# decadenza/SimpleStereo

Measured on AMD Instinct MI355X. Metric: disparity MPixels/s (H*W*nDisp per second), higher is better.
Workload: dtype f32

## Files before the change

simplestereo_amd/csrc/asw_pipe_kernel.hip.h:

```cpp
#pragma once
#include "asw_kernels.hip.h"
#ifndef SSAMD_KERNEL_TU
#include "lab_kernels.hip.h"
#endif

namespace ssamd {

#ifndef SSAMD_KERNEL_TU
static constexpr int TADV_COLS = 64;
template <bool BYTES>
__device__ __forceinline__ void asw_tad_tile(const void *__restrict__ srcL, const void *__restrict__ srcR, unsigned char *__restrict__ evol,
                                             int W, int pad, int minD, int Dc, int Se, int erow0, int erows, int evolW, int rd, long long npix_total,
                                             int bx, int by, int bz, char *smem)
{
    uint32_t *const sL = reinterpret_cast<uint32_t *>(smem);
    uint32_t *const sR = sL + TADV_COLS;
    const int r = erow0 + by, z = bz, uc0 = bx * TADV_COLS;
    const int P = Se >> 2, dlo = minD + z * Dc, dhi = dlo + Dc - 1;
    const int u0 = uc0 - pad, xr0 = u0 - dhi;
    auto pixel = [&](const void *src, int col) -> uint32_t {
        const size_t q = (size_t)r * W + col;
        if constexpr (BYTES) {
            typedef uint32_t __attribute__((aligned(1))) u32_unaligned;
            const uint8_t *const b = reinterpret_cast<const uint8_t *>(src) + 3 * q;
            return (long long)q + 1 < npix_total ? (*reinterpret_cast<const u32_unaligned *>(b) & 0xffffffu)
                                                 : ((uint32_t)b[0] | ((uint32_t)b[1] << 8) | ((uint32_t)b[2] << 16));
        } else {
            return reinterpret_cast<const PixRec *>(src)[q].bgrx;
        }
    };
    for (int k = threadIdx.x; k < 2 * TADV_COLS + Dc; k += blockDim.x) {
        const bool isL = k < TADV_COLS;
        const int col = isL ? u0 + k : xr0 + (k - TADV_COLS);
        const uint32_t v = (unsigned)col < (unsigned)W ? pixel(isL ? srcL : srcR, col) : 0x80000000u;
        (isL ? sL : sR)[isL ? k : k - TADV_COLS] = v;
    }
    __syncthreads();
    const int ncols = min(TADV_COLS, evolW - uc0);
    uint32_t *const out = reinterpret_cast<uint32_t *>(evol + (((size_t)z * erows + by) * (size_t)evolW + uc0) * Se);
    auto dword = [&](int c, int slot, uint32_t lp) {
        uint32_t v = 0;
        const int d0 = rd == 6 ? 6 * (slot >> 1) + 4 * (slot & 1) : 4 * slot, nv = rd == 6 && (slot & 1) ? 2 : 4;
        if (!(lp >> 31) && d0 < Dc) {
            const uint32_t *const rp = sR + c + (Dc - 1) - d0;
#pragma unroll
            for (int q = 0; q < 4; ++q) {
                const uint32_t rv = q < nv && d0 + q < Dc ? rp[-q] : 0x80000000u;
                if (!(rv >> 31)) v |= min(__builtin_amdgcn_sad_u8(lp, rv, 0u), 40u) << (8 * q);
            }
        }
        return v;
    };
    if ((P & 3) == 0) {
        const int P4 = P >> 2;
        uint4 *const out4 = reinterpret_cast<uint4 *>(out);
        for (int k = threadIdx.x; k < ncols * P4; k += blockDim.x) {
            const int c = k / P4, s4 = 4 * (k - c * P4);
            const uint32_t lp = sL[c];
            out4[k] = make_uint4(dword(c, s4, lp), dword(c, s4 + 1, lp), dword(c, s4 + 2, lp), dword(c, s4 + 3, lp));
        }
        return;
    }
    for (int k = threadIdx.x; k < ncols * P; k += blockDim.x) {
        const int c = k / P, slot = k - c * P;
        out[k] = dword(c, slot, sL[c]);
    }
}

__global__ __launch_bounds__(256) void asw_tad_volume_kernel(const PixRec *__restrict__ recL, const PixRec *__restrict__ recR,
                                                             unsigned char *__restrict__ evol, int W, int pad, int minD, int Dc,
                                                             int Se, int erow0, int erows, int evolW, int rd = 4)
{
    extern __shared__ __attribute__((aligned(16))) char smem[];
    asw_tad_tile<false>(recL, recR, evol, W, pad, minD, Dc, Se, erow0, erows, evolW, rd, 0, blockIdx.x, blockIdx.y, blockIdx.z, smem);
}

struct AswPrepassArgs {
    const uint8_t *bgrL, *bgrR;
    PixRec *recL, *recR;
    unsigned char *evol;
    long long npix_total;
    int W, pad, minD, Dc, Se, erow0, erows, evolW, rd;
    int lab_blocks, ex, ey;
};
__global__ __launch_bounds__(256) void asw_prepass_kernel(const AswPrepassArgs P)
{
    extern __shared__ __attribute__((aligned(16))) char smem[];
    if ((int)blockIdx.x < P.lab_blocks) {
        SSAMD_LAB_TABLES_IN_LDS(T)
        const long long np = (long long)P.erows * P.W, first = (long long)P.erow0 * P.W;
        const uint8_t *const bl = P.bgrL + 3 * first, *const br = P.bgrR + 3 * first;
        PixRec *const rl = P.recL + first, *const rr = P.recR + first;
        typedef uint32_t __attribute__((aligned(1))) u32_unaligned;
        for (long long q = (long long)blockIdx.x * blockDim.x + threadIdx.x; q < 2 * np; q += (long long)P.lab_blocks * blockDim.x) {
            const bool right = q >= np;
            const long long p = right ? q - np : q;
            const uint8_t *const bgr = right ? br : bl;
            uint32_t B, G, R;
            if (p + 1 < np) {
                const uint32_t v = *reinterpret_cast<const u32_unaligned *>(bgr + 3 * p);
                B = v & 0xff; G = (v >> 8) & 0xff; R = (v >> 16) & 0xff;
            } else {
                B = bgr[3 * p]; G = bgr[3 * p + 1]; R = bgr[3 * p + 2];
            }
            PixRec o;
            bgr_to_lab(B, G, R, o.L, o.a, o.b, T);
            o.bgrx = B | (G << 8) | (R << 16);
            (right ? rr : rl)[p] = o;
        }
        return;
    }
    const int b = (int)blockIdx.x - P.lab_blocks, bx = b % P.ex, by = (b / P.ex) % P.ey, bz = b / (P.ex * P.ey);
    asw_tad_tile<true>(P.bgrL, P.bgrR, P.evol, P.W, P.pad, P.minD, P.Dc, P.Se, P.erow0, P.erows, P.evolW, P.rd, P.npix_total, bx, by, bz, smem);
}

#endif

template <bool WITH_COSTS, int SLC = 0, int SRC = 0, int SEC = 0, bool CG = false>
__global__ __launch_bounds__(ASW_MAX_THREADS, 3) void asw_aggregate_pipe_kernel(const AswArgs A)
{
    constexpr bool STATIC = SLC > 0;
    static_assert(!CG || STATIC, "compile-time geometry belongs to a static tile");
    constexpr int RX = ASW_RX;
    constexpr int NWR = asw_nwr(RX);
    extern __shared__ __attribute__((aligned(16))) char smem[];
    constexpr AswGeom SG = asw_pipe_geom_constexpr(AswPipeTile<SLC, SRC, SEC>::id);
    static_assert(!STATIC || (SG.SL == SLC && SG.SR == SRC && SG.Se == SEC), "the strides name the tile");
    const AswGeom &g = CG ? SG : A.g;
    float *const wL = reinterpret_cast<float *>(smem + g.off_wL);
    float *const wR = reinterpret_cast<float *>(smem + g.off_wR);
    unsigned char *const eT0 = reinterpret_cast<unsigned char *>(smem + g.off_e);
    float4 *const labL = reinterpret_cast<float4 *>(smem + g.off_labL);
    float4 *const labR = reinterpret_cast<float4 *>(smem + g.off_labR);
    uint32_t *const bgrL = reinterpret_cast<uint32_t *>(smem + g.off_bgrL);
    uint32_t *const bgrR = reinterpret_cast<uint32_t *>(smem + g.off_bgrR);
    u64 *const bestL = reinterpret_cast<u64 *>(smem + g.off_bestL);
    u64 *const bestR = reinterpret_cast<u64 *>(smem + g.off_bestR);
    float4 *const cenLab = reinterpret_cast<float4 *>(smem + g.off_cen);
    float *const proxS = reinterpret_cast<float *>(smem + g.off_prox);

    const int tid = threadIdx.x, nthr = blockDim.x;
    const int W = A.W, win = CG ? AswPipeTile<SLC, SRC, SEC>::id.win : A.win, p = CG ? AswPipeTile<SLC, SRC, SEC>::id.win / 2 : A.pad;
    const int Tx = g.Tx, Dc = g.Dc, nL = g.nL, nR = g.nR, nRc = g.nRc, SR = g.SR, Se = g.Se;
    const int JC = g.JC, NC = g.NC;
    int bx = blockIdx.x;
    if ((gridDim.x & 7) == 0) bx = (bx & 7) * (gridDim.x >> 3) + (bx >> 3);
    const int x0 = bx * Tx;
    const int y = asw_out_row(A, blockIdx.y);
    const int dlo = A.minD + blockIdx.z * Dc;
    const int dhi = dlo + Dc - 1;
    if (min(x0 + Tx - 1, W - 1) - dlo < 0) {
        if (A.disp)
            for (int k = threadIdx.x; k < Tx && x0 + k < W; k += blockDim.x)
                A.disp[(size_t)(y - A.row0) * W + x0 + k] = (int16_t)(x0 + k);
        return;
    }
    const int segL_lo = x0 - p, xrc_lo = x0 - dhi, segR_lo = xrc_lo - p;
    const int phase = g.dephase ? __builtin_amdgcn_readfirstlane((int)(threadIdx.x >> 8)) : 1;

    float accN[RX][ASW_RD], accS[RX][ASW_RD];
#pragma unroll
    for (int a = 0; a < RX; ++a)
#pragma unroll
        for (int b = 0; b < ASW_RD; ++b) { accN[a][b] = 0.f; accS[a][b] = 0.f; }

    for (int k = tid; k < Tx; k += nthr) bestL[k] = KEY_NONE;
    for (int k = tid; k <= nRc; k += nthr) bestR[k] = KEY_NONE;
    for (int c = tid; c < Tx + nRc; c += nthr) {
        const bool isL = c < Tx;
        const int ccol = isL ? x0 + c : xrc_lo + (c - Tx);
        float4 v = make_float4(0.f, 0.f, 0.f, 0.f);
        if ((unsigned)ccol < (unsigned)W) {
            const PixRec q = (isL ? A.recL : A.recR)[(size_t)y * W + ccol];
            v = make_float4(q.L, q.a, q.b, 1.f);
        }
        cenLab[c] = v;
    }

    const int i_lo = max(0, p - y), i_hi = min(win, A.H + p - y);

    auto stage_row = [&](int i) {
        int tids = threadIdx.x;
        asm volatile("" : "+v"(tids));
        const int buf = i & 1, r = y - p + i;
        for (int k = tids; k < win; k += nthr) proxS[buf * win + k] = A.prox[i * win + k];
        const PixRec *const rowL = A.recL + (size_t)r * W;
        const PixRec *const rowR = A.recR + (size_t)r * W;
        for (int k = tids; k < nL + nR; k += nthr) {
            const bool isL = k < nL;
            const int idx = isL ? k : k - nL;
            const int col = (isL ? segL_lo : segR_lo) + idx;
            PixRec v;
            v.L = __builtin_inff();
            v.a = v.b = 0.f;
            v.bgrx = 0u;
            if ((unsigned)col < (unsigned)W) v = (isL ? rowL : rowR)[col];
            (isL ? labL + buf * nL : labR + buf * nR)[idx] = make_float4(v.L, v.a, v.b, 0.f);
            if (!A.evol) (isL ? bgrL + buf * nL : bgrR + buf * nR)[idx] = v.bgrx;
        }
    };
    auto build_e = [&](int i, int t_lo, int t_hi) {
        int tidb = threadIdx.x;
        asm volatile("" : "+v"(tidb));
        unsigned char *const eT = eT0 + (i & 1) * g.e_bytes;
        const uint32_t *const bgrLc = bgrL + (i & 1) * nL, *const bgrRc = bgrR + (i & 1) * nR;
        const int e_q = nthr / nL, e_r = nthr - e_q * nL;
        int t = t_lo + tidb;
        int sp = t / nL, ul = t - sp * nL;
        while (t < t_hi) {
            const uint32_t lp = bgrLc[ul];
            const uint32_t *const rp = bgrRc + (ul + (Dc - 1) - 8 * sp);
            uint32_t lo = 0, hi = 0;
#pragma unroll
            for (int k = 0; k < 4; ++k) {
                lo |= min(__builtin_amdgcn_sad_u8(lp, rp[-k], 0u), 40u) << (8 * k);
                hi |= min(__builtin_amdgcn_sad_u8(lp, rp[-4 - k], 0u), 40u) << (8 * k);
            }
            uint32_t *const dst = reinterpret_cast<uint32_t *>(eT + ul * Se) + 2 * sp;
            dst[0] = lo;
            if (2 * sp + 1 < g.DG) dst[1] = hi;
            t += nthr; ul += e_r; sp += e_q;
            if (ul >= nL) { ul -= nL; ++sp; }
        }
    };
    auto load_e = [&](int i) {
        int tidd = threadIdx.x;
        asm volatile("" : "+v"(tidd));
        const int r = y - p + i;
        const unsigned char *const src = A.evol + (((size_t)blockIdx.z * A.erows + (r - A.erow0)) * (size_t)A.evolW + x0) * Se;
        unsigned char *const dst = eT0 + (i & 1) * g.e_bytes;
        const int bytes = nL * Se, lane16 = (tidd & 63) * 16;
        for (int k = __builtin_amdgcn_readfirstlane(tidd >> 6) * 1024; k < bytes; k += (nthr >> 6) * 1024)
            if (k + lane16 < bytes)
                __builtin_amdgcn_global_load_lds((const void *)(src + k + lane16),
                                                 (__attribute__((address_space(3))) void *)(dst + k), 16, 0, 0);
    };
    auto build_weights = [&](int i, int jb, int je, int rb) {
        int tidw = threadIdx.x;
        asm volatile("" : "+v"(tidw));
        const float4 *const labLc = labL + (i & 1) * nL, *const labRc = labR + (i & 1) * nR;
        const float *const prow = proxS + (i & 1) * win;
        const int ncen = Tx + nRc;
        const int full = ncen / nthr * nthr, rest = ncen - full;
        int slen = je - jb, nseg = 1;
        if (rest > 0 && full > 0) {
            slen = max(ASW_WB, (je - jb + nthr / rest - 1) / (nthr / rest));
            slen = (slen + ASW_WB - 1) / ASW_WB * ASW_WB;
            nseg = (je - jb + slen - 1) / slen;
        }
        const int ntasks = full + rest * nseg;
        for (int t = tidw; t < ntasks; t += nthr) {
            int c = t, jb_t = jb, je_t = je;
            if (t >= full && nseg > 1) {
                const int q = t - full, sgm = q / rest;
                c = full + q - sgm * rest;
                jb_t = jb + sgm * slen;
                je_t = min(je, jb_t + slen);
            }
            const bool isL = c < Tx;
            const int cc = isL ? c : c - Tx;
            const float4 cen = cenLab[c];
            const float4 *const seg = (isL ? labLc : labRc) + cc;
            const int stride = isL ? g.SL : SR;
            float *const wout = (isL ? wL : wR) + cc + (rb - jb) * stride;
            int j = jb_t;
            const float4 *sp = seg + j;
            const float *pp = prow + j;
            float *wp = wout + j * stride;
            const int stride4 = ASW_WB * stride;
            for (; j + ASW_WB <= je_t; j += ASW_WB, sp += ASW_WB, pp += ASW_WB, wp += stride4) {
                float4 tp[ASW_WB];
                float pr[ASW_WB], wv[ASW_WB];
#pragma unroll
                for (int u = 0; u < ASW_WB; ++u) { tp[u] = sp[u]; pr[u] = pp[u]; }
#pragma unroll
                for (int u = 0; u < ASW_WB; ++u) {
                    asm volatile("" ::"v"(tp[u].w));
                    const float dL = tp[u].x - cen.x, da = tp[u].y - cen.y, db = tp[u].z - cen.z;
                    wv[u] = fmaf(db, db, fmaf(da, da, dL * dL));
                }
#pragma unroll
                for (int u = 0; u < ASW_WB; ++u) wv[u] = __builtin_amdgcn_sqrtf(wv[u]);
#pragma unroll
                for (int u = 0; u < ASW_WB; ++u) wv[u] = asw_weight_finish(wv[u], A.kC, pr[u]);
#pragma unroll
                for (int u = 0; u < ASW_WB; ++u) wp[u * stride] = wv[u];
            }
            if (j < je_t) {
                float4 tp[ASW_WB];
                float pr[ASW_WB], wv[ASW_WB];
#pragma unroll
                for (int u = 0; u < ASW_WB; ++u) {
                    const int jj = min(j + u, je_t - 1);
                    tp[u] = seg[jj];
                    pr[u] = prow[jj];
                }
#pragma unroll
                for (int u = 0; u < ASW_WB; ++u) {
                    asm volatile("" ::"v"(tp[u].w));
                    const float dL = tp[u].x - cen.x, da = tp[u].y - cen.y, db = tp[u].z - cen.z;
                    wv[u] = fmaf(db, db, fmaf(da, da, dL * dL));
                }
#pragma unroll
                for (int u = 0; u < ASW_WB; ++u) wv[u] = __builtin_amdgcn_sqrtf(wv[u]);
#pragma unroll
                for (int u = 0; u < ASW_WB; ++u) wv[u] = asw_weight_finish(wv[u], A.kC, pr[u]);
#pragma unroll
                for (int u = 0; u < ASW_WB; ++u) {
                    const int jj = min(j + u, je_t - 1);
                    wout[jj * stride] = wv[u];
                }
            }
        }
    };
    auto chunk_end = [&](int c) { return c == NC - 1 ? win : (c + 1) * JC; };
    const int nE = nL * ((g.DG + 1) >> 1);
    auto build_next = [&](int i, int c, int cb) {
        const bool more_rows = i + 1 < i_hi;
        if (c == 0 && more_rows) stage_row(i + 1);
        if (c == 0 && more_rows && A.evol) load_e(i + 1);
        if (c + 1 < NC) build_weights(i, (c + 1) * JC, chunk_end(c + 1), (cb ^ 1) * g.JCmax);
        else if (more_rows) build_weights(i + 1, 0, chunk_end(0), (cb ^ 1) * g.JCmax);
        if (c >= 1 && more_rows && !A.evol) build_e(i + 1, (int)((long long)nE * (c - 1) / (NC - 1)), (int)((long long)nE * c / (NC - 1)));
    };

    stage_row(i_lo);
    if (A.evol) load_e(i_lo);
    __syncthreads();
    if (!A.evol) build_e(i_lo, 0, nE);
    build_weights(i_lo, 0, chunk_end(0), 0);

    const int DGe = max(1, min(g.DG, (min(min(x0 + Tx, W) - 1, x0 + Tx - 1) - dlo) / ASW_RD + 1));
    const int nact = g.XG * DGe;
    int pk_xd;
    bool run;
    {
        const int tidm = threadIdx.x;
        int xg, dg;
        const int F = DGe >> 4, Lo = DGe & 15, nfull = g.XG * F;
        const int grp16 = tidm >> 4, r16 = tidm & 15;
        if (grp16 < nfull) {
            xg = grp16 / F;
            int gi = grp16 - xg * F;
            if (xg & 1) gi = F - 1 - gi;
            dg = 16 * gi + r16;
        } else {
            const int q = tidm - 16 * nfull;
            xg = Lo ? q / Lo : g.XG;
            dg = 16 * F + (Lo ? q - xg * Lo : 0);
        }
        pk_xd = xg | (dg << 16);
        const bool tile_live = tidm < nact && x0 + RX * xg < W && dlo + ASW_RD * dg <= A.maxD &&
                               x0 + RX * xg + RX - 1 - (dlo + ASW_RD * dg) >= 0;
        run = __builtin_amdgcn_ballot_w64(tile_live) != 0 && tidm < nact;
    }

    int cb = 0;
#pragma nounroll
    for (int i = i_lo; i < i_hi; ++i) {
        const unsigned char *const eT = eT0 + (i & 1) * g.e_bytes;
        AswRow ew[RX];

#pragma nounroll
        for (int c = 0; c < NC; ++c) {
            __syncthreads();
            const int jc = c * JC, jend = chunk_end(c);
            const int rb = cb * g.JCmax;
            if (phase == 0) build_next(i, c, cb);
            if (run) {
                const int xg = pk_xd & 0xffff, dg = pk_xd >> 16;
                const unsigned char *erow = eT + (RX * xg + (jc == 0 ? 0 : RX - 1 + jc)) * Se + 4 * dg;
                if (jc == 0) {
#pragma unroll
                    for (int n = 0; n < RX - 1; ++n) {
                        asw_row_unpack(ew[n], *reinterpret_cast<const uint32_t *>(erow));
                        erow += Se;
                    }
                }
                const float *wlp = wL + rb * g.SL + 8 * xg;
                const float *wrp = wR + rb * SR + (RX * xg - ASW_RD * dg + Dc - ASW_RD);
                for (int j0 = jc; j0 < jend; j0 += RX) {
#define SSAMD_PSTEP(JJ)                                                                             \
    if (j0 + (JJ) < jend) {                                                                         \
        const uint32_t epk = *reinterpret_cast<const uint32_t *>(erow + (STATIC ? (JJ) * SEC : 0)); \
        if constexpr (!STATIC) erow += Se;                                                          \
        float wl[RX], wr[NWR];                                                                      \
        {                                                                                           \
            const float *const wl_ = wlp + (STATIC ? (JJ) * SLC : 0);                              \
            const float *const wr_ = wrp + (STATIC ? (JJ) * SRC : 0);                              \
            const float4 v0 = *reinterpret_cast<const float4 *>(wl_);                              \
            wl[0] = v0.x; wl[1] = v0.y; wl[2] = v0.z; wl[3] = v0.w;                                 \
            const float4 v1 = *reinterpret_cast<const float4 *>(wl_ + 4);                          \
            wl[4] = v1.x; wl[5] = v1.y; wl[6] = v1.z; wl[7] = v1.w;                                 \
            const float4 r0 = *reinterpret_cast<const float4 *>(wr_);                              \
            const float4 r1 = *reinterpret_cast<const float4 *>(wr_ + 4);                          \
            const float4 r2 = *reinterpret_cast<const float4 *>(wr_ + 8);                          \
            asm volatile("" ::"v"(r2.w));       \
            wr[0] = r0.x; wr[1] = r0.y; wr[2] = r0.z; wr[3] = r0.w;                                 \
            wr[4] = r1.x; wr[5] = r1.y; wr[6] = r1.z; wr[7] = r1.w;                                 \
            wr[8] = r2.x; wr[9] = r2.y; wr[10] = r2.z; wr[11] = r2.w;                               \
        }                                                                                           \
        if constexpr (!STATIC) { wlp += g.SL; wrp += SR; }                                         \
               \
        _Pragma("unroll") for (int xi = 0; xi < RX; ++xi) {                                         \
            if (xi == RX - 1) asw_row_unpack(ew[((JJ) + RX - 1) % RX], epk);                        \
            const AswRow &row_ = ew[((JJ) + xi) % RX];                                              \
            _Pragma("unroll") for (int di = 0; di < ASW_RD; ++di) {                                 \
                const float w_ = wl[xi] * wr[xi - di + ASW_RD - 1];                                 \
                accN[xi][di] = fmaf(w_, row_.e[di], accN[xi][di]);                                  \
                accS[xi][di] = fmaf(w_, row_.c[di], accS[xi][di]);                                  \
            }                                                                                       \
        }                                                                                           \
    }
                    SSAMD_PSTEP(0) SSAMD_PSTEP(1) SSAMD_PSTEP(2) SSAMD_PSTEP(3)
                    SSAMD_PSTEP(4) SSAMD_PSTEP(5) SSAMD_PSTEP(6) SSAMD_PSTEP(7)
#undef SSAMD_PSTEP
                    if constexpr (STATIC) { erow += RX * SEC; wlp += RX * SLC; wrp += RX * SRC; }
                }
            }
            if (phase != 0) build_next(i, c, cb);
            cb ^= 1;
        }
    }

    int tidf = threadIdx.x;
    asm volatile("" : "+v"(tidf));
#define ASW_EPI_RD ASW_RD
#define ASW_EPI_LIVE (tidf < nact)
#define ASW_EPI_XG(live) (pk_xd & 0xffff)
#define ASW_EPI_DG(live) (pk_xd >> 16)
#define ASW_EPI_TX Tx
#define ASW_EPI_NRC nRc
#define ASW_EPI_TID tid
#define ASW_EPI_NTHR nthr
#define ASW_EPI_SYNC() __syncthreads()
#define ASW_EPI_ROW (size_t)(y - A.row0) * W
#include "asw_epilogue.inc"
}

}
```

Baseline: 10650.

## Assign weight-build work per wavefront and read proximity weights from constant memory

Weight construction now distributes whole 64-lane wavefront columns of centres (left and right separately) instead of flat thread tasks. This keeps left/right branching uniform per wave, uses compile-time strides for static tiles and replaces the clamped remainder with exact 1-3 element batches. The proximity row is no longer staged into shared memory. It is read directly through the constant address space (scalar loads), which removes an LDS copy per row. The risks are heavier integer loop bookkeeping for task splitting and possibly worse load balance when the centre count does not fill the waves.

```diff
diff --git a/simplestereo_amd/csrc/asw_pipe_kernel.hip.h b/simplestereo_amd/csrc/asw_pipe_kernel.hip.h
--- a/simplestereo_amd/csrc/asw_pipe_kernel.hip.h
+++ b/simplestereo_amd/csrc/asw_pipe_kernel.hip.h
@@ -137,7 +137,6 @@
     u64 *const bestL = reinterpret_cast<u64 *>(smem + g.off_bestL);
     u64 *const bestR = reinterpret_cast<u64 *>(smem + g.off_bestR);
     float4 *const cenLab = reinterpret_cast<float4 *>(smem + g.off_cen);
-    float *const proxS = reinterpret_cast<float *>(smem + g.off_prox);
 
     const int tid = threadIdx.x, nthr = blockDim.x;
     const int W = A.W, win = CG ? AswPipeTile<SLC, SRC, SEC>::id.win : A.win, p = CG ? AswPipeTile<SLC, SRC, SEC>::id.win / 2 : A.pad;
@@ -183,7 +182,6 @@
         int tids = threadIdx.x;
         asm volatile("" : "+v"(tids));
         const int buf = i & 1, r = y - p + i;
-        for (int k = tids; k < win; k += nthr) proxS[buf * win + k] = A.prox[i * win + k];
         const PixRec *const rowL = A.recL + (size_t)r * W;
         const PixRec *const rowR = A.recR + (size_t)r * W;
         for (int k = tids; k < nL + nR; k += nthr) {
@@ -236,81 +234,75 @@
                                                  (__attribute__((address_space(3))) void *)(dst + k), 16, 0, 0);
     };
     auto build_weights = [&](int i, int jb, int je, int rb) {
+        static_assert(ASW_WB == 4, "the remainder below is written out for batches of four");
+        typedef const __attribute__((address_space(4))) float cfloat;
         int tidw = threadIdx.x;
         asm volatile("" : "+v"(tidw));
+        const int wave = __builtin_amdgcn_readfirstlane(tidw >> 6), lane = tidw & 63;
+        constexpr int NTHR = STATIC ? asw_cx_round_up((SLC / ASW_RX) * ((SRC - SLC) / ASW_RD), 64) : 0;
+        static_assert(!STATIC || (SG.Tx == SLC && SG.nRc == SRC - 1 && SG.threads == NTHR), "the strides name the centres and the threads");
+        const int TxB = STATIC ? SLC : Tx, nRcB = STATIC ? SRC - 1 : nRc, nw = (STATIC ? NTHR : nthr) >> 6;
+        const int nLw = (TxB + 63) >> 6, ncw = nLw + ((nRcB + 63) >> 6);
         const float4 *const labLc = labL + (i & 1) * nL, *const labRc = labR + (i & 1) * nR;
-        const float *const prow = proxS + (i & 1) * win;
-        const int ncen = Tx + nRc;
-        const int full = ncen / nthr * nthr, rest = ncen - full;
+        cfloat *const prow = reinterpret_cast<cfloat *>(reinterpret_cast<uintptr_t>(A.prox)) + i * win;
+        auto batch = [&](auto n_, const float4 &cen, const float4 *sp, cfloat *pp, float *wp, int stride) {
+            constexpr int N = decltype(n_)::value;
+            float4 tp[N];
+            float pr[N], wv[N];
+#pragma unroll
+            for (int u = 0; u < N; ++u) { tp[u] = sp[u]; pr[u] = pp[u]; }
+#pragma unroll
+            for (int u = 0; u < N; ++u) {
+                asm volatile("" ::"v"(tp[u].w));
+                const float dL = tp[u].x - cen.x, da = tp[u].y - cen.y, db = tp[u].z - cen.z;
+                wv[u] = fmaf(db, db, fmaf(da, da, dL * dL));
+            }
+#pragma unroll
+            for (int u = 0; u < N; ++u) wv[u] = __builtin_amdgcn_sqrtf(wv[u]);
+#pragma unroll
+            for (int u = 0; u < N; ++u) wv[u] = asw_weight_finish(wv[u], A.kC, pr[u]);
+#pragma unroll
+            for (int u = 0; u < N; ++u) wp[u * stride] = wv[u];
+        };
+        auto build_side = [&](auto left_, int cc, int jb_t, int je_t) {
+            constexpr bool LEFT = decltype(left_)::value;
+            const int stride = LEFT ? (STATIC ? SLC : g.SL) : (STATIC ? SRC : SR);
+            if (cc >= (LEFT ? TxB : nRcB)) return;
+            const float4 cen = cenLab[(LEFT ? 0 : TxB) + cc];
+            asm volatile("" ::"v"(cen.w));
+            const float4 *sp = (LEFT ? labLc : labRc) + cc + jb_t;
+            cfloat *pp = prow + jb_t;
+            float *wp = (LEFT ? wL : wR) + cc + (rb + jb_t - jb) * stride;
+            int j = jb_t;
+#pragma nounroll
+            for (; j + ASW_WB <= je_t; j += ASW_WB, sp += ASW_WB, pp += ASW_WB, wp += ASW_WB * stride)
+                batch(std::integral_constant<int, ASW_WB>{}, cen, sp, pp, wp, stride);
+            const int rem = je_t - j;
+            if (rem == 1) batch(std::integral_constant<int, 1>{}, cen, sp, pp, wp, stride);
+            else if (rem == 2) batch(std::integral_constant<int, 2>{}, cen, sp, pp, wp, stride);
+            else if (rem == 3) batch(std::integral_constant<int, 3>{}, cen, sp, pp, wp, stride);
+        };
+        int full = 0;
+        while (full + nw <= ncw) full += nw;
+        const int rest = ncw - full;
         int slen = je - jb, nseg = 1;
         if (rest > 0 && full > 0) {
-            slen = max(ASW_WB, (je - jb + nthr / rest - 1) / (nthr / rest));
-            slen = (slen + ASW_WB - 1) / ASW_WB * ASW_WB;
-            nseg = (je - jb + slen - 1) / slen;
-        }
-        const int ntasks = full + rest * nseg;
-        for (int t = tidw; t < ntasks; t += nthr) {
-            int c = t, jb_t = jb, je_t = je;
+            int per = 0;
+            for (int a = rest; a <= nw; a += rest) ++per;
+            for (slen = ASW_WB; slen * per < je - jb;) slen += ASW_WB;
+            while (nseg * slen < je - jb) ++nseg;
+        }
+        for (int t = wave; t < full + rest * nseg; t += nw) {
+            int cw = t, jb_t = jb, je_t = je;
             if (t >= full && nseg > 1) {
-                const int q = t - full, sgm = q / rest;
-                c = full + q - sgm * rest;
+                int q = t - full, sgm = 0;
+                while (q >= rest) { q -= rest; ++sgm; }
+                cw = full + q;
                 jb_t = jb + sgm * slen;
                 je_t = min(je, jb_t + slen);
             }
-            const bool isL = c < Tx;
-            const int cc = isL ? c : c - Tx;
-            const float4 cen = cenLab[c];
-            const float4 *const seg = (isL ? labLc : labRc) + cc;
-            const int stride = isL ? g.SL : SR;
-            float *const wout = (isL ? wL : wR) + cc + (rb - jb) * stride;
-            int j = jb_t;
-            const float4 *sp = seg + j;
-            const float *pp = prow + j;
-            float *wp = wout + j * stride;
-            const int stride4 = ASW_WB * stride;
-            for (; j + ASW_WB <= je_t; j += ASW_WB, sp += ASW_WB, pp += ASW_WB, wp += stride4) {
-                float4 tp[ASW_WB];
-                float pr[ASW_WB], wv[ASW_WB];
-#pragma unroll
-                for (int u = 0; u < ASW_WB; ++u) { tp[u] = sp[u]; pr[u] = pp[u]; }
-#pragma unroll
-                for (int u = 0; u < ASW_WB; ++u) {
-                    asm volatile("" ::"v"(tp[u].w));
-                    const float dL = tp[u].x - cen.x, da = tp[u].y - cen.y, db = tp[u].z - cen.z;
-                    wv[u] = fmaf(db, db, fmaf(da, da, dL * dL));
-                }
-#pragma unroll
-                for (int u = 0; u < ASW_WB; ++u) wv[u] = __builtin_amdgcn_sqrtf(wv[u]);
-#pragma unroll
-                for (int u = 0; u < ASW_WB; ++u) wv[u] = asw_weight_finish(wv[u], A.kC, pr[u]);
-#pragma unroll
-                for (int u = 0; u < ASW_WB; ++u) wp[u * stride] = wv[u];
-            }
-            if (j < je_t) {
-                float4 tp[ASW_WB];
-                float pr[ASW_WB], wv[ASW_WB];
-#pragma unroll
-                for (int u = 0; u < ASW_WB; ++u) {
-                    const int jj = min(j + u, je_t - 1);
-                    tp[u] = seg[jj];
-                    pr[u] = prow[jj];
-                }
-#pragma unroll
-                for (int u = 0; u < ASW_WB; ++u) {
-                    asm volatile("" ::"v"(tp[u].w));
-                    const float dL = tp[u].x - cen.x, da = tp[u].y - cen.y, db = tp[u].z - cen.z;
-                    wv[u] = fmaf(db, db, fmaf(da, da, dL * dL));
-                }
-#pragma unroll
-                for (int u = 0; u < ASW_WB; ++u) wv[u] = __builtin_amdgcn_sqrtf(wv[u]);
-#pragma unroll
-                for (int u = 0; u < ASW_WB; ++u) wv[u] = asw_weight_finish(wv[u], A.kC, pr[u]);
-#pragma unroll
-                for (int u = 0; u < ASW_WB; ++u) {
-                    const int jj = min(j + u, je_t - 1);
-                    wout[jj * stride] = wv[u];
-                }
-            }
+            if (cw < nLw) build_side(std::true_type{}, 64 * cw + lane, jb_t, je_t);
+            else build_side(std::false_type{}, 64 * (cw - nLw) + lane, jb_t, je_t);
         }
     };
     auto chunk_end = [&](int c) { return c == NC - 1 ? win : (c + 1) * JC; };
@@ -319,8 +311,10 @@
         const bool more_rows = i + 1 < i_hi;
         if (c == 0 && more_rows) stage_row(i + 1);
         if (c == 0 && more_rows && A.evol) load_e(i + 1);
-        if (c + 1 < NC) build_weights(i, (c + 1) * JC, chunk_end(c + 1), (cb ^ 1) * g.JCmax);
-        else if (more_rows) build_weights(i + 1, 0, chunk_end(0), (cb ^ 1) * g.JCmax);
+        if (c + 1 < NC || more_rows) {
+            const int cn = c + 1 < NC ? c + 1 : 0;
+            build_weights(c + 1 < NC ? i : i + 1, cn * JC, chunk_end(cn), (cb ^ 1) * g.JCmax);
+        }
         if (c >= 1 && more_rows && !A.evol) build_e(i + 1, (int)((long long)nE * (c - 1) / (NC - 1)), (int)((long long)nE * c / (NC - 1)));
     };
 
```

Result: faster. 10780, median of 6 (+1.2%).
